# maxwerhahn/Multi-pass-GAN

Measured on AMD Instinct MI355X. Metric: volumes/sec (4x two-pass generator inference, 64^3->256^3 density-only), higher is better.
Workload: dtype f16+2xbf6->f32

## Files before the change

### include/mpgan.h

```cpp
#ifndef MPGAN_H
#define MPGAN_H

#include <stddef.h>
#include <stdint.h>

#ifdef __cplusplus
extern "C" {
#endif

typedef void* mpg_stream_t;

enum { MPG_OK = 0, MPG_ERR_ARG = 1, MPG_ERR_HIP = 2, MPG_ERR_UNSUPPORTED = 3 };

enum { MPG_ACT_NONE = 0, MPG_ACT_RELU = 1, MPG_ACT_LRELU = 2, MPG_ACT_TANH = 3 };

enum { MPG_PREC_F16X1 = 1, MPG_PREC_F16F6 = 2, MPG_PREC_F16X3 = 3 };

enum { MPG_G8_F16 = 0 };

const char* mpg_last_error(void);
int mpg_device_info(int* cu_count, char* arch_name, int arch_name_len);
const char* mpg_version(void);

size_t mpg_g8_bytes(int n, int h, int w, int c);
// ... 31 lines not shown
    float*  y;
    void*   y_g8;
    int32_t prec;
    int32_t reserved;
    const float* in_amax;
} mpg_conv_desc;

size_t mpg_conv_pack_size(int kh, int kw, int cin, int cout, int prec);

int mpg_conv_pack_weights(mpg_stream_t stream, const float* w_hwio, int kh, int kw,
                          int w_cin_total, int w_c_off, int cin, int cout,
                          float wscale, const float* cout_scale,
                          int prec, void* out, size_t out_bytes);

int mpg_conv2d_fused(mpg_stream_t stream, const mpg_conv_desc* desc);

int mpg_conv2d_fused_d2s(mpg_stream_t stream, const mpg_conv_desc* desc, int r, int c_total, int co_off);

int mpg_conv2d_fused_window(mpg_stream_t stream, const mpg_conv_desc* desc, int c_total, int co_off);

typedef struct mpg_small_pair_desc {
    int32_t n, h, w;
    const void* x;
    int32_t cin, cgroups, g_off, up_log2;
    const void* wpack_a;
    int32_t kh_a, kw_a, cmid;
    const float* bias_a;
    int32_t act_a;
    float   leak_a;
    const void* wpack_b;
// ... 179 lines not shown
```

### multi-pass-gan_amd/_lib.py

```python
import ctypes
import os

_HERE = os.path.dirname(os.path.abspath(__file__))
LIB_PATH = os.path.join(_HERE, "csrc", "libmpgan_hip.so")
if os.environ.get("MPGAN_LIB_OVERRIDE"):
    LIB_PATH = os.path.abspath(os.environ["MPGAN_LIB_OVERRIDE"])

MPG_OK = 0
ACT_NONE, ACT_RELU, ACT_LRELU, ACT_TANH = 0, 1, 2, 3
PREC_F16X1, PREC_F16F6, PREC_F16X3 = 1, 2, 3
G8_F16 = 0
MAX_SEG = 4
WGRAD_PLAN_INTS, WGRAD_FORM_ROW, WGRAD_FORM_RING = 24, 0, 1
DEFLATE_UNIT, DEFLATE_SLOT, DEFLATE_SLAB = 32768, 32768 + 16, 64 << 20

_ACT_IDS = {None: ACT_NONE, "none": ACT_NONE, "relu": ACT_RELU, "lrelu": ACT_LRELU, "tanh": ACT_TANH}


def act_id(name):
    try:
        return _ACT_IDS[name]
    except KeyError:
        raise ValueError("unknown activation %r" % (name,))


class MpgError(RuntimeError):
    pass

# ... 63 lines not shown
_Z = ctypes.c_size_t
_F = ctypes.c_float

PROTOTYPES = {
    "mpg_last_error": (ctypes.c_char_p, []),
    "mpg_version": (ctypes.c_char_p, []),
    "mpg_device_info": (_I, [ctypes.POINTER(_I), ctypes.c_char_p, _I]),
    "mpg_g8_bytes": (_Z, [_I, _I, _I, _I]),
    "mpg_f32_to_g8": (_I, [_P, _P, _I, _I, _I, _I, _I, _I, _I, _P]),
    "mpg_f32_to_g8_scaled": (_I, [_P, _P, _I, _I, _I, _I, _I, _I, _I, _P, _P]),
    "mpg_absmax": (_I, [_P, _P, _Z, _P]),
    "mpg_g8_to_f32": (_I, [_P, _P, _I, _I, _I, _I, _P]),
    "mpg_conv_pack_size": (_Z, [_I, _I, _I, _I, _I]),
    "mpg_conv_pack_weights": (_I, [_P, _P, _I, _I, _I, _I, _I, _I, _F, _P, _I, _P, _Z]),
    "mpg_conv2d_fused": (_I, [_P, ctypes.POINTER(ConvDesc)]),
    "mpg_conv2d_fused_d2s": (_I, [_P, ctypes.POINTER(ConvDesc), _I, _I, _I]),
    "mpg_conv2d_fused_window": (_I, [_P, ctypes.POINTER(ConvDesc), _I, _I]),
    "mpg_conv2d_small_pair": (_I, [_P, ctypes.POINTER(SmallPairDesc)]),
    "mpg_conv2d_direct": (_I, [_P, _P, _I, _I, _I, _I, _P, _I, _I, _I, _I, _I, _F, _P, _P, _I, _F, _P]),
    "mpg_resize_nearest": (_I, [_P, _P, _I, _I, _I, _I, _P, _I, _I]),
    "mpg_resize_bilinear": (_I, [_P, _P, _I, _I, _I, _I, _P, _I, _I]),
    "mpg_resize_bicubic": (_I, [_P, _P, _I, _I, _I, _I, _P, _I, _I]),
    "mpg_avg_pool2": (_I, [_P, _P, _I, _I, _I, _I, _P]),
    "mpg_max_pool": (_I, [_P, _P, _I, _I, _I, _I, _I, _I, _P, _P]),
    "mpg_max_pool_bwd": (_I, [_P, _P, _P, _I, _I, _I, _I, _I, _I, _P]),
    "mpg_pixel_norm": (_I, [_P, _P, _Z, _I, _F, _P]),
    "mpg_pixel_norm_g8": (_I, [_P, _P, _I, _I, _I, _I, _F, _P]),
    "mpg_minibatch_stddev": (_I, [_P, _P, _I, _I, _I, _I, _I, _P, _P]),
    "mpg_minibatch_stddev_bwd": (_I, [_P, _P, _P, _I, _I, _I, _I, _I, _P, _P]),
    "mpg_minibatch_stddev_bwd2": (_I, [_P, _P, _P, _P, _I, _I, _I, _I, _I, _P, _P, _P, _Z]),
# ... 94 lines not shown
```

### multi-pass-gan_amd/csrc/mpgan_conv.h

```cpp
#pragma once
#include "mpgan_internal.h"
#include "mpgan_mfma_dev.h"

namespace mpg::conv {

using namespace mpg::dev;

constexpr int TW = 32;
constexpr int TAPOFF_BYTES = 1024;
constexpr int epi_rowf(int nt) { return nt * 32 + 4; }

struct SegArgs {
    const char* x;
    const char* w;
    int cg_seg;
    int cg_total, g_off;
    int kh, kw;
    int up, upy;
    int cgc, nchunks, sc;
    int ih, iw;
    int pt, pl;
    int hs, ws;
    int np;
    int ni_img;
// ... 22 lines not shown
    int tap_bytes;
    int tiles_x, tiles_y;
    int dbg;
};

typedef const __attribute__((address_space(4))) ConvArgs* KArgs;

struct ConvArgsD2S {
    ConvArgs a;
    int cs;
    int coff;
    int cg;
};
typedef const __attribute__((address_space(4))) ConvArgsD2S* KArgsD2S;

template <bool D2S>
struct KernelArgs { typedef ConvArgs type; };
template <>
struct KernelArgs<true> { typedef ConvArgsD2S type; };

struct D2SPos {
    int cc;
    size_t pix;
};
__device__ __forceinline__ D2SPos d2s_pos(const KArgsD2S dp, int py, int px, int c) {
    const int gc = dp->coff + c;
    const int k = gc / dp->cs;
    D2SPos p;
    p.cc = gc - k * dp->cs;
    p.pix = (size_t)(2 * py + (k >> 1)) * (2 * dp->a.w) + 2 * px + (k & 1);
// ... 64 lines not shown
            const int c = (k >> 2) * 8 + 4 * hh + (k & 3);
            stg_lane[c] = c < cout ? tanhf(stg_lane[c]) : 0.f;
        }
#pragma unroll
        for (int nt = 0; nt < NT; ++nt)
#pragma unroll
            for (int q4 = 0; q4 < 4; ++q4) {
                const float4 v = *reinterpret_cast<const float4*>(stg_lane + nt * 32 + 8 * q4 + 4 * hh);
                acc[nt][4 * q4] = v.x;
                acc[nt][4 * q4 + 1] = v.y;
                acc[nt][4 * q4 + 2] = v.z;
                acc[nt][4 * q4 + 3] = v.w;
            }
        return;
    }
    float4 bq[2][4];
#pragma unroll
    for (int q4 = 0; q4 < 4; ++q4) bq[0][q4] = *reinterpret_cast<const float4*>(bl + 8 * q4 + 4 * hh);
#pragma unroll
    for (int nt = 0; nt < NT; ++nt) {
        if (nt + 1 < NT) {
#pragma unroll
            for (int q4 = 0; q4 < 4; ++q4) bq[(nt + 1) & 1][q4] = *reinterpret_cast<const float4*>(bl + (nt + 1) * 32 + 8 * q4 + 4 * hh);
        }
        __builtin_amdgcn_sched_barrier(0);
#pragma unroll
        for (int q4 = 0; q4 < 4; ++q4) {
            const int co0 = nt * 32 + 8 * q4 + 4 * hh;
            const float b4[4] = {bq[nt & 1][q4].x, bq[nt & 1][q4].y, bq[nt & 1][q4].z, bq[nt & 1][q4].w};
#pragma unroll
            for (int i = 0; i < 4; ++i) {
                float v = mpg::apply_act(acc[nt][4 * q4 + i] * unscale + b4[i], ACT, leak);
                if (co0 + i >= cout) v = 0.f;
                acc[nt][4 * q4 + i] = v;
            }
        }
        __builtin_amdgcn_sched_barrier(0);
    }
}

template <int NT>
__device__ __forceinline__ void epilogue_row_values(f32x16 (&acc)[NT], const KArgs ap, const float* bl, float* stg_lane, float unscale,
                                                    int hh) {
    const auto& a = *ap;
    switch (a.act) {
        case MPG_ACT_RELU: epilogue_bias_act<MPG_ACT_RELU>(acc, bl, stg_lane, unscale, a.leak, a.cout, hh); break;
        case MPG_ACT_LRELU: epilogue_bias_act<MPG_ACT_LRELU>(acc, bl, stg_lane, unscale, a.leak, a.cout, hh); break;
        case MPG_ACT_TANH: epilogue_bias_act<MPG_ACT_TANH>(acc, bl, stg_lane, unscale, a.leak, a.cout, hh); break;
        default: epilogue_bias_act<MPG_ACT_NONE>(acc, bl, stg_lane, unscale, a.leak, a.cout, hh); break;
    }
    if (a.pn) {
        float ss = 0.f;
#pragma unroll
        for (int nt = 0; nt < NT; ++nt)
#pragma unroll
            for (int i = 0; i < 16; ++i) ss += acc[nt][i] * acc[nt][i];
        ss += __shfl_xor(ss, 32);
        const float sc = rsqrtf(ss / (float)a.cout + a.pn_eps);
#pragma unroll
        for (int nt = 0; nt < NT; ++nt)
#pragma unroll
            for (int i = 0; i < 16; ++i) acc[nt][i] *= sc;
    }
}

template <int NT, int PT, bool D2S = false>
__device__ __forceinline__ void conv_epilogue(f32x16 (&acc)[PT][NT], const KArgs ap, char* smem, int n, int y0, int x0,
                                              int wave, int lane, const EpiPre pre) {
    const auto& a = *ap;
    const KArgsD2S dp = reinterpret_cast<KArgsD2S>(ap);
    const int r = lane & 31;
    const int hh = lane >> 5;
    constexpr int ROWF = epi_rowf(NT);
    static_assert(128 * sizeof(float) <= TAPOFF_BYTES, "the staged bias must fit in front of the staging rows");
    float* bl = reinterpret_cast<float*>(smem);
    float* stg = reinterpret_cast<float*>(smem + TAPOFF_BYTES) + wave * (32 * ROWF);
    const int cg_out = (a.cout + 7) >> 3;
    const float unscale = 1.f / mpg::pow2_scale(pre.amax);
    {
        float bv = pre.bias;
        asm volatile("" : "+v"(bv));
        if (wave < 2) bl[wave * 64 + lane] = bv;
    }
    __syncthreads();
    const int npx = min(32, a.w - x0);
    const size_t plane_px = (size_t)a.h * a.w;
    if (a.y == nullptr && a.post_add == nullptr) {
#pragma unroll
        for (int pt = 0; pt < PT; ++pt) {
            const int py = y0 + PT * wave + pt;
            epilogue_row_values<NT>(acc[pt], ap, bl, stg + r * ROWF, unscale, hh);
            if (py < a.h && r < npx && !(a.dbg & 2)) {
#pragma unroll
                for (int nt = 0; nt < NT; ++nt)
#pragma unroll
                    for (int qp = 0; qp < 2; ++qp) {
                        float v[8];
#pragma unroll
                        for (int i = 0; i < 4; ++i) {
                            typedef unsigned v2u_t __attribute__((ext_vector_type(2)));
                            const v2u_t sw = __builtin_amdgcn_permlane32_swap(__float_as_uint(acc[pt][nt][8 * qp + i]),
                                                                              __float_as_uint(acc[pt][nt][8 * qp + 4 + i]), false, false);
                            v[i] = __uint_as_float(sw[0]);
                            v[4 + i] = __uint_as_float(sw[1]);
                        }
                        const int cg = nt * 4 + 2 * qp + hh;
                        if (cg < cg_out) {
                            char* dst;
                            size_t plane_out = plane_px;
                            if constexpr (D2S) {
                                const D2SPos q = d2s_pos(dp, py, x0 + r, 8 * cg);
                                plane_out = 4 * plane_px;
                                dst = a.y_g8 + ((((size_t)n * dp->cg + (q.cc >> 3)) * 2) * plane_out + q.pix) * 16;
                            } else {
                                dst = a.y_g8 + ((((size_t)n * a.cg_img + cg) * 2) * plane_px + (size_t)py * a.w + x0 + r) * 16;
                            }
                            half8 hi, lo;
#pragma unroll
                            for (int j = 0; j < 8; ++j) {
                                hi[j] = (_Float16)v[j];
                                lo[j] = (_Float16)(v[j] - (float)hi[j]);
                            }
                            __builtin_nontemporal_store(hi, reinterpret_cast<half8*>(dst));
                            __builtin_nontemporal_store(lo, reinterpret_cast<half8*>(dst + plane_out * 16));
                        }
                    }
            }
        }
        return;
    }
#pragma unroll
    for (int pt = 0; pt < PT; ++pt) {
        const int py = y0 + PT * wave + pt;
        epilogue_row_values<NT>(acc[pt], ap, bl, stg + r * ROWF, unscale, hh);
#pragma unroll
        for (int nt = 0; nt < NT; ++nt)
#pragma unroll
            for (int q4 = 0; q4 < 4; ++q4) {
                const int co0 = nt * 32 + 8 * q4 + 4 * hh;
                *reinterpret_cast<float4*>(stg + r * ROWF + co0) =
                    make_float4(acc[pt][nt][4 * q4], acc[pt][nt][4 * q4 + 1], acc[pt][nt][4 * q4 + 2], acc[pt][nt][4 * q4 + 3]);
            }
        if (py < a.h && !(a.dbg & 2)) {
// ... 99 lines not shown
    int slots;
    int stages;
};
SegShape seg_shape(int kh, int kw, int cin, int nt, int prec);

constexpr size_t LDS_MAX = 160 * 1024;

size_t pack_base_bytes(int kh, int kw, int cin, int cout, int prec);
inline bool small_layer(int cin, int cout) { return cin <= 8 && cout <= 8; }
inline int pad_before(int k, int pad_hi) { return pad_hi ? k / 2 : (k - 1) / 2; }
int check_segment(const mpg_conv_desc* d, int s);

hipError_t launch_conv_f16(int prec, int nt, dim3 grid, size_t lds, hipStream_t st, const ConvArgs& a);
hipError_t launch_conv_f16(int prec, int nt, dim3 grid, size_t lds, hipStream_t st, const ConvArgsD2S& a);
hipError_t launch_conv_f6(int nt, dim3 grid, size_t lds, hipStream_t st, const ConvArgs& a);
int launch_small(hipStream_t stream, const mpg_conv_desc* d);

}
```

### multi-pass-gan_amd/csrc/mpgan_conv_mfma.hip

```cpp
#include "mpgan_conv.h"

using namespace mpg::conv;

namespace {

template <class P>
constexpr Shape shape_of() {
    return {P::TH, P::KS, P::WAVES, P::WSTAGE, P::R * P::WSTAGE, P::ROWF};
}
constexpr Shape SHAPES[3][4] = {
    {shape_of<Pipe<1, 1>>(), shape_of<Pipe<2, 1>>(), shape_of<Pipe<3, 1>>(), shape_of<Pipe<4, 1>>()},
    {shape_of<Pipe6<1>>(), shape_of<Pipe6<2>>(), shape_of<Pipe6<3>>(), shape_of<Pipe6<4>>()},
    {shape_of<Pipe<1, 3>>(), shape_of<Pipe<2, 3>>(), shape_of<Pipe<3, 3>>(), shape_of<Pipe<4, 3>>()},
};
static_assert(MPG_PREC_F16X1 == 1 && MPG_PREC_F16F6 == 2 && MPG_PREC_F16X3 == 3, "SHAPES is indexed by prec - 1");

constexpr size_t LDS_TWO_WG = 80 * 1024;
struct LdsPlan {
    size_t tap, loop, epi, total;
};
LdsPlan lds_plan(int tap_slots, int img_bytes, const Shape& ps) {
    LdsPlan l;
    l.tap = ((size_t)tap_slots * 4 + 1023) / 1024 * 1024;
    if (l.tap < (size_t)TAPOFF_BYTES) l.tap = TAPOFF_BYTES;
// ... 27 lines not shown
    s.stages = s.sc = (s.nchunks * s.tp + stage_slots - 1) / stage_slots;
    s.slots = s.sc * stage_slots;
    s.pref = 1;
    for (int g = 1; g < s.nchunks; ++g)
        if ((g * s.tp) / stage_slots - ((g - 1) * s.tp + stage_slots - 1) / stage_slots < 2) s.pref = 0;
    return s;
}

struct D2SOut {
    int cs, coff;
};

struct WinOut {
    int c_total, co_off;
};

}

const Shape& mpg::conv::pipe_shape(int nt, int prec) { return SHAPES[prec - 1][nt - 1]; }

SegShape mpg::conv::seg_shape(int kh, int kw, int cin, int nt, int prec) {
    if (prec == MPG_PREC_F16F6) return seg_shape_f6(kh, kw, cin, nt);
    const Shape& ps = pipe_shape(nt, prec);
    const int cg = (cin + 7) / 8;
    SegShape s = {};
    set_image(s, ps, kh, kw, 2);
    if (cg < 2 || !((kh * kw) & 1) || lds_plan(0, s.img_bytes, ps).loop > LDS_TWO_WG) set_image(s, ps, kh, kw, 1);
    s.nchunks = (cg + s.cgc - 1) / s.cgc;
    const int ksteps = (kh * kw * s.cgc + 1) / 2;
    s.sc = (ksteps + ps.ks - 1) / ps.ks;
// ... 13 lines not shown

int mpg::conv::check_segment(const mpg_conv_desc* d, int s) {
    const mpg_conv_seg& g = d->seg[s];
    MPG_REQUIRE(g.x && g.wpack, "mpg_conv2d_fused: segment %d null pointer", s);
    MPG_REQUIRE(g.kh >= 1 && g.kh <= 7 && g.kw >= 1 && g.kw <= 7, "mpg_conv2d_fused: segment %d kernel %dx%d", s, g.kh, g.kw);
    MPG_REQUIRE(g.cin >= 1 && g.g_off >= 0 && g.g_off + (g.cin + 7) / 8 <= g.cgroups,
                "mpg_conv2d_fused: segment %d channel-group range", s);
    MPG_REQUIRE(g.up_log2 >= 0 && g.up_log2 <= 4, "mpg_conv2d_fused: segment %d up_log2 %d", s, g.up_log2);
    MPG_REQUIRE(g.up_x_only == 0 || g.up_x_only == 1, "mpg_conv2d_fused: segment %d up_x_only %d (0 or 1)", s, g.up_x_only);
    MPG_REQUIRE((g.up_x_only || (d->h % (1 << g.up_log2)) == 0) && (d->w % (1 << g.up_log2)) == 0,
                "mpg_conv2d_fused: segment %d: %dx%d not divisible by upsample %d", s, d->h, d->w, 1 << g.up_log2);
    MPG_REQUIRE((((uintptr_t)g.x) & 15) == 0 && (((uintptr_t)g.wpack) & 15) == 0, "mpg_conv2d_fused: segment %d misaligned", s);
    return MPG_OK;
}

static int launch_mfma(hipStream_t stream, const mpg_conv_desc* d, const D2SOut* d2s, const WinOut& win) {
    const int nt = (d->cout + 31) / 32;
    const Shape& ps = pipe_shape(nt, d->prec);
    ConvArgs a;
    a.n = d->n; a.h = d->h; a.w = d->w; a.cout = d->cout; a.nseg = d->nseg;
    int max_img = 0, max_slots = 0;
    for (int s = 0; s < d->nseg; ++s) {
        if (const int rc = check_segment(d, s)) return rc;
        const mpg_conv_seg& g = d->seg[s];
        const SegShape ss = seg_shape(g.kh, g.kw, g.cin, nt, d->prec);
        MPG_REQUIRE(d->prec == MPG_PREC_F16F6 || ss.slots <= TAPOFF_BYTES / 4, "mpg_conv2d_fused: segment %d tap table too large", s);
        SegArgs& o = a.seg[s];
        o.x = (const char*)g.x; o.w = (const char*)g.wpack;
        o.cg_seg = (g.cin + 7) / 8; o.cg_total = g.cgroups; o.g_off = g.g_off;
        o.kh = g.kh; o.kw = g.kw; o.up = g.up_log2; o.upy = g.up_x_only ? 0 : g.up_log2;
        o.cgc = ss.cgc; o.nchunks = ss.nchunks; o.sc = ss.sc;
        o.ih = ps.th + g.kh - 1; o.iw = TW + g.kw - 1;
        o.pt = pad_before(g.kh, g.pad_hi); o.pl = pad_before(g.kw, g.pad_hi);
        o.hs = d->h >> o.upy; o.ws = d->w >> o.up;
        o.np = ss.np; o.ni_img = ss.ni_img;
        o.direct = ss.direct;
        o.tp = ss.tp;
        MPG_REQUIRE(!ss.direct || (size_t)o.hs * o.ws * 16 * 16 < ((size_t)1 << 31),
                    "mpg_conv2d_fused: segment %d: %dx%d too large for the 1x1 path (32-bit group offsets)", s, d->h, d->w);
        o.pref = ss.pref;
// ... 6 lines not shown
    MPG_REQUIRE(!d->post_add || d->post_add_coff + d->cout <= d->post_add_stride, "mpg_conv2d_fused: post_add channel range");
    a.y_stride = win.c_total;
    a.cg_img = (win.c_total + 7) / 8;
    a.y = d->y != nullptr ? d->y + win.co_off : nullptr;
    a.y_g8 = d->y_g8 != nullptr ? (char*)d->y_g8 + (size_t)(win.co_off / 8) * 2 * d->h * d->w * 16 : nullptr;
    MPG_REQUIRE((((uintptr_t)d->y) & 15) == 0 && (((uintptr_t)d->y_g8) & 15) == 0,
                "mpg_conv2d_fused: misaligned output");
    a.zeros = mpg::zero_page();
    MPG_REQUIRE(a.zeros != nullptr, "mpg_conv2d_fused: could not allocate the zero page");
    a.img_bytes = max_img;
    a.tiles_x = (d->w + TW - 1) / TW;
    a.tiles_y = (d->h + ps.th - 1) / ps.th;
    a.dbg = d->reserved;
    const long nblk = (long)d->n * a.tiles_x * a.tiles_y;
    MPG_REQUIRE(nblk < (1L << 31), "mpg_conv2d_fused: grid too large");
    const LdsPlan lds = lds_plan(max_slots, max_img, ps);
    a.tap_bytes = (int)lds.tap;
    MPG_REQUIRE(lds.total <= LDS_MAX, "mpg_conv2d_fused: LDS budget %zu exceeds 160 KiB", lds.total);
    const dim3 grid((unsigned)nblk);
    hipError_t le;
    if (d2s != nullptr) {
        ConvArgsD2S ad;
        ad.a = a;
        ad.cs = d2s->cs;
        ad.coff = d2s->coff;
        ad.cg = d2s->cs / 8;
        le = launch_conv_f16(d->prec, nt, grid, lds.total, stream, ad);
    } else if (d->prec == MPG_PREC_F16F6) {
        le = launch_conv_f6(nt, grid, lds.total, stream, a);
    } else {
        le = launch_conv_f16(d->prec, nt, grid, lds.total, stream, a);
    }
    if (le != hipSuccess) return mpg::hip_check(le, "mpg_conv2d_fused: hipFuncSetAttribute(dynamic LDS)");
    MPG_LAUNCH_CHECK("conv_mfma_kernel");
}

static int conv2d_fused(mpg_stream_t stream, const mpg_conv_desc* d, const D2SOut* d2s, const WinOut* window = nullptr) {
    MPG_REQUIRE(d != nullptr, "mpg_conv2d_fused: null desc");
    MPG_REQUIRE(d->n >= 1 && d->h >= 1 && d->w >= 1, "mpg_conv2d_fused: bad shape %d x %d x %d", d->n, d->h, d->w);
    MPG_REQUIRE(d->cout >= 1 && d->cout <= 128, "mpg_conv2d_fused: cout %d not in 1..128", d->cout);
    MPG_REQUIRE(d->nseg >= 1 && d->nseg <= MPG_MAX_SEG, "mpg_conv2d_fused: nseg %d", d->nseg);
    MPG_REQUIRE(d->y != nullptr || d->y_g8 != nullptr, "mpg_conv2d_fused: no output requested");
    MPG_REQUIRE(d->prec == MPG_PREC_F16X1 || d->prec == MPG_PREC_F16X3 || d->prec == MPG_PREC_F16F6,
                "mpg_conv2d_fused: bad prec %d", d->prec);
    MPG_REQUIRE(d->act >= MPG_ACT_NONE && d->act <= MPG_ACT_TANH, "mpg_conv2d_fused: bad act %d", d->act);
    bool small = d->cout <= 8 && !d->pixel_norm && d->post_add == nullptr && d->reserved == 0 && d2s == nullptr && window == nullptr;
    for (int s = 0; s < d->nseg && small; ++s) small = d->seg[s].cin <= 8;
    const WinOut whole = {d->cout, 0};
    return small ? launch_small((hipStream_t)stream, d) : launch_mfma((hipStream_t)stream, d, d2s, window != nullptr ? *window : whole);
}

extern "C" int mpg_conv2d_fused(mpg_stream_t stream, const mpg_conv_desc* d) {
    return conv2d_fused(stream, d, nullptr);
}

extern "C" int mpg_conv2d_fused_d2s(mpg_stream_t stream, const mpg_conv_desc* d, int r, int c_total, int co_off) {
    MPG_REQUIRE(d != nullptr, "mpg_conv2d_fused_d2s: null desc");
    MPG_REQUIRE(r == 2, "mpg_conv2d_fused_d2s: block size %d (only 2)", r);
    MPG_REQUIRE(c_total >= 4 && c_total % 4 == 0, "mpg_conv2d_fused_d2s: %d channels are not a multiple of 4", c_total);
    MPG_REQUIRE(co_off >= 0 && d->cout >= 1 && co_off + d->cout <= c_total,
                "mpg_conv2d_fused_d2s: channels [%d, %d) outside 0..%d", co_off, co_off + d->cout, c_total);
    MPG_REQUIRE(!d->pixel_norm && d->post_add == nullptr, "mpg_conv2d_fused_d2s: no pixel norm or post-add");
    if (d->prec == MPG_PREC_F16F6) {
        mpg::set_error("mpg_conv2d_fused_d2s: MPG_PREC_F16F6 has no depth-to-space store (use MPG_PREC_F16X3 / F16X1)");
// ... 23 lines not shown
```

### multi-pass-gan_amd/csrc/mpgan_mfma_dev.h

```cpp
#pragma once
#include <hip/hip_runtime.h>
#include <type_traits>

namespace mpg::dev {

typedef _Float16 half8 __attribute__((ext_vector_type(8)));
typedef float f32x16 __attribute__((ext_vector_type(16)));

typedef int v4i __attribute__((ext_vector_type(4)));

template <int N>
__device__ __forceinline__ void wait_dma_and_barrier() {
    asm volatile("s_waitcnt vmcnt(%0) lgkmcnt(0)\n\ts_barrier" ::"n"(N) : "memory");
}
__device__ __forceinline__ void wait_dma_late_and_barrier(int late) {
    asm volatile(
        "s_cmp_lt_u32 %0, 1\n\t"
        "s_cbranch_scc1 .Lmpg_w0_%=\n\t"
        "s_cmp_lt_u32 %0, 2\n\t"
        "s_cbranch_scc1 .Lmpg_w1_%=\n\t"
        "s_cmp_lt_u32 %0, 3\n\t"
        "s_cbranch_scc1 .Lmpg_w2_%=\n\t"
        "s_cmp_lt_u32 %0, 4\n\t"
        "s_cbranch_scc1 .Lmpg_w3_%=\n\t"
// ... 50 lines not shown
```

### multi-pass-gan_amd/ops.py

```python
import ctypes

import torch

from . import _lib
from ._lib import G8_F16, PREC_F16F6, PREC_F16X1, PREC_F16X3

DEFAULT_PREC = PREC_F16X3
INFERENCE_PREC = PREC_F16F6
F16F6_MIN_K = 256


def parse_prec(v):
    names = {"f16f6": PREC_F16F6, "f16x3": PREC_F16X3, "f16x1": PREC_F16X1, "fp32": PREC_F16X3}
    s = str(v).strip().lower()
    if s in names:
        return names[s]
    try:
        p = int(s)
    except ValueError:
        p = -1
    if p not in (PREC_F16X1, PREC_F16F6, PREC_F16X3):
        raise _lib.MpgError("prec %r: expected 1 (f16x1), 2 (f16f6) or 3 (f16x3)" % (v,))
    return p

# ... 176 lines not shown
                 in_amax=None):
    lib = _lib.load()
    d = _conv_desc(segments, out_hw, _dev(bias, "bias") if bias is not None else None, act, leak)
    shape = (d.n, d.h, d.w, d.cout)
    d.pixel_norm, d.pn_eps = int(bool(pixel_norm)), pn_eps
    if post_add is not None:
        pa = _checked_post_add(post_add, post_add_coff, shape, "conv2d_fused")
        d.post_add, d.post_add_stride, d.post_add_coff = pa.data_ptr(), pa.shape[3], post_add_coff
    y, y8, outs = _alloc_outputs(shape, segments[0].x.buf.device, want_f32, want_g8, out, "conv2d_fused")
    d.y, d.y_g8 = _ptr(y), _ptr(y8)
    d.reserved = reserved
    if in_amax is not None:
        d.in_amax = _dev(in_amax, "in_amax").data_ptr()
    _lib.check(lib.mpg_conv2d_fused(_stream(), ctypes.byref(d)), "mpg_conv2d_fused")
    return outs[0] if len(outs) == 1 else tuple(outs)


def _launch_windows(what, entry, lead_args, chunks, out_hw, c_total, out_c, bias, act, leak, want_f32, want_g8, out,
                    post_add=None, post_add_coff=0, g8_only=False):
    lib = _lib.load()
    if not chunks:
        raise _lib.MpgError("%s: no chunks" % what)
    co = 0
    for segments, co_off in sorted(chunks, key=lambda ch: ch[1]):
        if co_off != co:
            break
        co += segments[0].packed.cout
    if co != c_total:
        raise _lib.MpgError("%s: the chunks do not cover channels 0..%d once" % (what, c_total))
    if bias is not None:
# ... 504 lines not shown
```

Measured before the change: 15.68.

## Add persistent resident conv kernel with atomic tile scheduler and double-buffered images

Adds a persistent conv kernel launched with one block per compute unit. Each block pulls output tiles from a global atomic counter and double-buffers the input image tile in LDS, so the DMA for the next tile overlaps the MFMA work and epilogue of the current one. The kernel is used automatically for single-segment f16x1/f16x3 convolutions with 96-128 output channels, g8-only output and no tanh or post-add. It also factors the g8 epilogue into a shared helper and exposes plan/kernel-selection entry points for testing. In exchange it adds per-stream counter state that must reset correctly between launches, and a smaller grid that relies on the dynamic scheduler to balance load.

```diff
diff --git a/include/mpgan.h b/include/mpgan.h
--- a/include/mpgan.h
+++ b/include/mpgan.h
@@ -69,6 +69,13 @@
                           int prec, void* out, size_t out_bytes);
 
 int mpg_conv2d_fused(mpg_stream_t stream, const mpg_conv_desc* desc);
+
+#define MPG_CONV_PLAN_INTS 8
+#define MPG_CONV_KERNEL_SMALL 0
+#define MPG_CONV_KERNEL_STREAM 1
+#define MPG_CONV_KERNEL_RESIDENT 2
+int mpg_conv2d_fused_plan(const mpg_conv_desc* desc, int d2s, int32_t* record);
+int mpg_conv2d_fused_kernel(mpg_stream_t stream, const mpg_conv_desc* desc, int kernel, int blocks);
 
 int mpg_conv2d_fused_d2s(mpg_stream_t stream, const mpg_conv_desc* desc, int r, int c_total, int co_off);
 
diff --git a/multi-pass-gan_amd/_lib.py b/multi-pass-gan_amd/_lib.py
--- a/multi-pass-gan_amd/_lib.py
+++ b/multi-pass-gan_amd/_lib.py
@@ -12,6 +12,7 @@
 G8_F16 = 0
 MAX_SEG = 4
 WGRAD_PLAN_INTS, WGRAD_FORM_ROW, WGRAD_FORM_RING = 24, 0, 1
+CONV_PLAN_INTS, CONV_KERNEL_SMALL, CONV_KERNEL_STREAM, CONV_KERNEL_RESIDENT = 8, 0, 1, 2
 DEFLATE_UNIT, DEFLATE_SLOT, DEFLATE_SLAB = 32768, 32768 + 16, 64 << 20
 
 _ACT_IDS = {None: ACT_NONE, "none": ACT_NONE, "relu": ACT_RELU, "lrelu": ACT_LRELU, "tanh": ACT_TANH}
@@ -105,6 +106,8 @@
     "mpg_conv_pack_size": (_Z, [_I, _I, _I, _I, _I]),
     "mpg_conv_pack_weights": (_I, [_P, _P, _I, _I, _I, _I, _I, _I, _F, _P, _I, _P, _Z]),
     "mpg_conv2d_fused": (_I, [_P, ctypes.POINTER(ConvDesc)]),
+    "mpg_conv2d_fused_plan": (_I, [ctypes.POINTER(ConvDesc), _I, ctypes.POINTER(ctypes.c_int32)]),
+    "mpg_conv2d_fused_kernel": (_I, [_P, ctypes.POINTER(ConvDesc), _I, _I]),
     "mpg_conv2d_fused_d2s": (_I, [_P, ctypes.POINTER(ConvDesc), _I, _I, _I]),
     "mpg_conv2d_fused_window": (_I, [_P, ctypes.POINTER(ConvDesc), _I, _I]),
     "mpg_conv2d_small_pair": (_I, [_P, ctypes.POINTER(SmallPairDesc)]),
diff --git a/multi-pass-gan_amd/csrc/mpgan_conv.h b/multi-pass-gan_amd/csrc/mpgan_conv.h
--- a/multi-pass-gan_amd/csrc/mpgan_conv.h
+++ b/multi-pass-gan_amd/csrc/mpgan_conv.h
@@ -60,6 +60,14 @@
 };
 typedef const __attribute__((address_space(4))) ConvArgsD2S* KArgsD2S;
 
+struct ConvArgsRes {
+    ConvArgs a;
+    unsigned* ctr;
+    int ntiles;
+    int nblocks;
+};
+typedef const __attribute__((address_space(4))) ConvArgsRes* KArgsRes;
+
 template <bool D2S>
 struct KernelArgs { typedef ConvArgs type; };
 template <>
@@ -154,14 +162,14 @@
             }
         return;
     }
-    float4 bq[2][4];
-#pragma unroll
-    for (int q4 = 0; q4 < 4; ++q4) bq[0][q4] = *reinterpret_cast<const float4*>(bl + 8 * q4 + 4 * hh);
+    v4f bq[2][4];
+#pragma unroll
+    for (int q4 = 0; q4 < 4; ++q4) bq[0][q4] = *reinterpret_cast<const v4f*>(bl + 8 * q4 + 4 * hh);
 #pragma unroll
     for (int nt = 0; nt < NT; ++nt) {
         if (nt + 1 < NT) {
 #pragma unroll
-            for (int q4 = 0; q4 < 4; ++q4) bq[(nt + 1) & 1][q4] = *reinterpret_cast<const float4*>(bl + (nt + 1) * 32 + 8 * q4 + 4 * hh);
+            for (int q4 = 0; q4 < 4; ++q4) bq[(nt + 1) & 1][q4] = *reinterpret_cast<const v4f*>(bl + (nt + 1) * 32 + 8 * q4 + 4 * hh);
         }
         __builtin_amdgcn_sched_barrier(0);
 #pragma unroll
@@ -179,14 +187,18 @@
     }
 }
 
-template <int NT>
+template <int NT, bool TANH = true>
 __device__ __forceinline__ void epilogue_row_values(f32x16 (&acc)[NT], const KArgs ap, const float* bl, float* stg_lane, float unscale,
                                                     int hh) {
     const auto& a = *ap;
     switch (a.act) {
         case MPG_ACT_RELU: epilogue_bias_act<MPG_ACT_RELU>(acc, bl, stg_lane, unscale, a.leak, a.cout, hh); break;
         case MPG_ACT_LRELU: epilogue_bias_act<MPG_ACT_LRELU>(acc, bl, stg_lane, unscale, a.leak, a.cout, hh); break;
-        case MPG_ACT_TANH: epilogue_bias_act<MPG_ACT_TANH>(acc, bl, stg_lane, unscale, a.leak, a.cout, hh); break;
+        case MPG_ACT_TANH:
+            if constexpr (TANH) {
+                epilogue_bias_act<MPG_ACT_TANH>(acc, bl, stg_lane, unscale, a.leak, a.cout, hh);
+                break;
+            }
         default: epilogue_bias_act<MPG_ACT_NONE>(acc, bl, stg_lane, unscale, a.leak, a.cout, hh); break;
     }
     if (a.pn) {
@@ -201,6 +213,61 @@
         for (int nt = 0; nt < NT; ++nt)
 #pragma unroll
             for (int i = 0; i < 16; ++i) acc[nt][i] *= sc;
+    }
+}
+
+constexpr int epilogue_g8_stores(int nt, int pt) { return pt * nt * 2 * 2; }
+template <int NT, int PT, bool D2S = false, bool TANH = true>
+__device__ __forceinline__ void epilogue_rows_g8(f32x16 (&acc)[PT][NT], const KArgs ap, const float* bl, float* stg, int n, int y0,
+                                                 int x0, int wave, int lane, float unscale) {
+    const auto& a = *ap;
+    const KArgsD2S dp = reinterpret_cast<KArgsD2S>(ap);
+    const int r = lane & 31;
+    const int hh = lane >> 5;
+    constexpr int ROWF = epi_rowf(NT);
+    const int cg_out = (a.cout + 7) >> 3;
+    const int npx = min(32, a.w - x0);
+    const size_t plane_px = (size_t)a.h * a.w;
+#pragma unroll
+    for (int pt = 0; pt < PT; ++pt) {
+        const int py = y0 + PT * wave + pt;
+        epilogue_row_values<NT, TANH>(acc[pt], ap, bl, stg + r * ROWF, unscale, hh);
+        if (py < a.h && r < npx && !(a.dbg & 2)) {
+#pragma unroll
+            for (int nt = 0; nt < NT; ++nt)
+#pragma unroll
+                for (int qp = 0; qp < 2; ++qp) {
+                    float v[8];
+#pragma unroll
+                    for (int i = 0; i < 4; ++i) {
+                        typedef unsigned v2u_t __attribute__((ext_vector_type(2)));
+                        const v2u_t sw = __builtin_amdgcn_permlane32_swap(__float_as_uint(acc[pt][nt][8 * qp + i]),
+                                                                          __float_as_uint(acc[pt][nt][8 * qp + 4 + i]), false, false);
+                        v[i] = __uint_as_float(sw[0]);
+                        v[4 + i] = __uint_as_float(sw[1]);
+                    }
+                    const int cg = nt * 4 + 2 * qp + hh;
+                    if (cg < cg_out) {
+                        char* dst;
+                        size_t plane_out = plane_px;
+                        if constexpr (D2S) {
+                            const D2SPos q = d2s_pos(dp, py, x0 + r, 8 * cg);
+                            plane_out = 4 * plane_px;
+                            dst = a.y_g8 + ((((size_t)n * dp->cg + (q.cc >> 3)) * 2) * plane_out + q.pix) * 16;
+                        } else {
+                            dst = a.y_g8 + ((((size_t)n * a.cg_img + cg) * 2) * plane_px + (size_t)py * a.w + x0 + r) * 16;
+                        }
+                        half8 hi, lo;
+#pragma unroll
+                        for (int j = 0; j < 8; ++j) {
+                            hi[j] = (_Float16)v[j];
+                            lo[j] = (_Float16)(v[j] - (float)hi[j]);
+                        }
+                        __builtin_nontemporal_store(hi, reinterpret_cast<half8*>(dst));
+                        __builtin_nontemporal_store(lo, reinterpret_cast<half8*>(dst + plane_out * 16));
+                    }
+                }
+        }
     }
 }
 
@@ -226,47 +293,7 @@
     const int npx = min(32, a.w - x0);
     const size_t plane_px = (size_t)a.h * a.w;
     if (a.y == nullptr && a.post_add == nullptr) {
-#pragma unroll
-        for (int pt = 0; pt < PT; ++pt) {
-            const int py = y0 + PT * wave + pt;
-            epilogue_row_values<NT>(acc[pt], ap, bl, stg + r * ROWF, unscale, hh);
-            if (py < a.h && r < npx && !(a.dbg & 2)) {
-#pragma unroll
-                for (int nt = 0; nt < NT; ++nt)
-#pragma unroll
-                    for (int qp = 0; qp < 2; ++qp) {
-                        float v[8];
-#pragma unroll
-                        for (int i = 0; i < 4; ++i) {
-                            typedef unsigned v2u_t __attribute__((ext_vector_type(2)));
-                            const v2u_t sw = __builtin_amdgcn_permlane32_swap(__float_as_uint(acc[pt][nt][8 * qp + i]),
-                                                                              __float_as_uint(acc[pt][nt][8 * qp + 4 + i]), false, false);
-                            v[i] = __uint_as_float(sw[0]);
-                            v[4 + i] = __uint_as_float(sw[1]);
-                        }
-                        const int cg = nt * 4 + 2 * qp + hh;
-                        if (cg < cg_out) {
-                            char* dst;
-                            size_t plane_out = plane_px;
-                            if constexpr (D2S) {
-                                const D2SPos q = d2s_pos(dp, py, x0 + r, 8 * cg);
-                                plane_out = 4 * plane_px;
-                                dst = a.y_g8 + ((((size_t)n * dp->cg + (q.cc >> 3)) * 2) * plane_out + q.pix) * 16;
-                            } else {
-                                dst = a.y_g8 + ((((size_t)n * a.cg_img + cg) * 2) * plane_px + (size_t)py * a.w + x0 + r) * 16;
-                            }
-                            half8 hi, lo;
-#pragma unroll
-                            for (int j = 0; j < 8; ++j) {
-                                hi[j] = (_Float16)v[j];
-                                lo[j] = (_Float16)(v[j] - (float)hi[j]);
-                            }
-                            __builtin_nontemporal_store(hi, reinterpret_cast<half8*>(dst));
-                            __builtin_nontemporal_store(lo, reinterpret_cast<half8*>(dst + plane_out * 16));
-                        }
-                    }
-            }
-        }
+        epilogue_rows_g8<NT, PT, D2S>(acc, ap, bl, stg, n, y0, x0, wave, lane, unscale);
         return;
     }
 #pragma unroll
@@ -396,6 +423,10 @@
 hipError_t launch_conv_f16(int prec, int nt, dim3 grid, size_t lds, hipStream_t st, const ConvArgs& a);
 hipError_t launch_conv_f16(int prec, int nt, dim3 grid, size_t lds, hipStream_t st, const ConvArgsD2S& a);
 hipError_t launch_conv_f6(int nt, dim3 grid, size_t lds, hipStream_t st, const ConvArgs& a);
+constexpr int RES_TH = 16, RES_WAVES = 8, RES_CTL_BYTES = 1024;
+unsigned* resident_counters(hipStream_t st);
+int resident_default_blocks();
+hipError_t launch_conv_resident(int prec, int nt, size_t lds, hipStream_t st, const ConvArgsRes& a);
 int launch_small(hipStream_t stream, const mpg_conv_desc* d);
 
 }
diff --git a/multi-pass-gan_amd/csrc/mpgan_conv_mfma.hip b/multi-pass-gan_amd/csrc/mpgan_conv_mfma.hip
--- a/multi-pass-gan_amd/csrc/mpgan_conv_mfma.hip
+++ b/multi-pass-gan_amd/csrc/mpgan_conv_mfma.hip
@@ -65,6 +65,37 @@
 struct WinOut {
     int c_total, co_off;
 };
+
+constexpr int ROUTE_AUTO = -1;
+
+bool small_launch(const mpg_conv_desc* d, bool d2s, bool window) {
+    bool small = d->cout <= 8 && !d->pixel_norm && d->post_add == nullptr && d->reserved == 0 && !d2s && !window;
+    for (int s = 0; s < d->nseg && small; ++s) small = d->seg[s].cin <= 8;
+    return small;
+}
+
+struct ResidentPlan {
+    bool ok;
+    SegShape ss;
+    size_t lds;
+};
+ResidentPlan resident_plan(const mpg_conv_desc* d, bool d2s) {
+    ResidentPlan p = {};
+    const int nt = (d->cout + 31) / 32;
+    if ((d->prec != MPG_PREC_F16X3 && d->prec != MPG_PREC_F16X1) || d->nseg != 1 || d2s || nt < 3 || nt > 4) return p;
+    if (d->y != nullptr || d->y_g8 == nullptr || d->post_add != nullptr || d->act == MPG_ACT_TANH) return p;
+    const mpg_conv_seg& g = d->seg[0];
+    if (g.kh < 1 || g.kh > 7 || g.kw < 1 || g.kw > 7 || g.cin < 1) return p;
+    p.ss = seg_shape(g.kh, g.kw, g.cin, nt, d->prec);
+    if (p.ss.nchunks != 1 || p.ss.slots > TAPOFF_BYTES / 4) return p;
+    Shape tile = pipe_shape(nt, d->prec);
+    tile.th = RES_TH;
+    tile.waves = RES_WAVES;
+    set_image(p.ss, tile, g.kh, g.kw, p.ss.cgc);
+    p.lds = (size_t)TAPOFF_BYTES + RES_CTL_BYTES + (size_t)p.ss.stages * tile.wstage + 2 * (size_t)p.ss.img_bytes;
+    p.ok = p.lds <= LDS_MAX;
+    return p;
+}
 
 }
 
@@ -108,16 +139,26 @@
     return MPG_OK;
 }
 
-static int launch_mfma(hipStream_t stream, const mpg_conv_desc* d, const D2SOut* d2s, const WinOut& win) {
+static int launch_mfma(hipStream_t stream, const mpg_conv_desc* d, const D2SOut* d2s, const WinOut& win, int route = ROUTE_AUTO,
+                       int blocks = 0) {
     const int nt = (d->cout + 31) / 32;
-    const Shape& ps = pipe_shape(nt, d->prec);
+    const ResidentPlan rplan = route == MPG_CONV_KERNEL_STREAM ? ResidentPlan{} : resident_plan(d, d2s != nullptr);
+    MPG_REQUIRE(route != MPG_CONV_KERNEL_RESIDENT || rplan.ok, "mpg_conv2d_fused_kernel: the launch is not eligible for conv_resident_kernel");
+    unsigned* ctr = rplan.ok ? resident_counters(stream) : nullptr;
+    MPG_REQUIRE(route != MPG_CONV_KERNEL_RESIDENT || ctr != nullptr, "mpg_conv2d_fused_kernel: no counter slot for this stream");
+    const bool resident = ctr != nullptr;
+    Shape ps = pipe_shape(nt, d->prec);
+    if (resident) {
+        ps.th = RES_TH;
+        ps.waves = RES_WAVES;
+    }
     ConvArgs a;
     a.n = d->n; a.h = d->h; a.w = d->w; a.cout = d->cout; a.nseg = d->nseg;
     int max_img = 0, max_slots = 0;
     for (int s = 0; s < d->nseg; ++s) {
         if (const int rc = check_segment(d, s)) return rc;
         const mpg_conv_seg& g = d->seg[s];
-        const SegShape ss = seg_shape(g.kh, g.kw, g.cin, nt, d->prec);
+        const SegShape ss = resident ? rplan.ss : seg_shape(g.kh, g.kw, g.cin, nt, d->prec);
         MPG_REQUIRE(d->prec == MPG_PREC_F16F6 || ss.slots <= TAPOFF_BYTES / 4, "mpg_conv2d_fused: segment %d tap table too large", s);
         SegArgs& o = a.seg[s];
         o.x = (const char*)g.x; o.w = (const char*)g.wpack;
@@ -154,6 +195,19 @@
     a.dbg = d->reserved;
     const long nblk = (long)d->n * a.tiles_x * a.tiles_y;
     MPG_REQUIRE(nblk < (1L << 31), "mpg_conv2d_fused: grid too large");
+    if (resident) {
+        ConvArgsRes ar;
+        ar.a = a;
+        ar.a.tap_bytes = TAPOFF_BYTES;
+        ar.ctr = ctr;
+        ar.ntiles = (int)nblk;
+        if (blocks <= 0) blocks = resident_default_blocks();
+        MPG_REQUIRE(blocks > 0, "mpg_conv2d_fused: could not read the device's compute-unit count");
+        ar.nblocks = blocks > nblk ? (int)nblk : blocks;
+        const hipError_t e = launch_conv_resident(d->prec, nt, rplan.lds, stream, ar);
+        if (e != hipSuccess) return mpg::hip_check(e, "mpg_conv2d_fused: hipFuncSetAttribute(dynamic LDS)");
+        MPG_LAUNCH_CHECK("conv_resident_kernel");
+    }
     const LdsPlan lds = lds_plan(max_slots, max_img, ps);
     a.tap_bytes = (int)lds.tap;
     MPG_REQUIRE(lds.total <= LDS_MAX, "mpg_conv2d_fused: LDS budget %zu exceeds 160 KiB", lds.total);
@@ -175,7 +229,7 @@
     MPG_LAUNCH_CHECK("conv_mfma_kernel");
 }
 
-static int conv2d_fused(mpg_stream_t stream, const mpg_conv_desc* d, const D2SOut* d2s, const WinOut* window = nullptr) {
+static int check_desc(const mpg_conv_desc* d) {
     MPG_REQUIRE(d != nullptr, "mpg_conv2d_fused: null desc");
     MPG_REQUIRE(d->n >= 1 && d->h >= 1 && d->w >= 1, "mpg_conv2d_fused: bad shape %d x %d x %d", d->n, d->h, d->w);
     MPG_REQUIRE(d->cout >= 1 && d->cout <= 128, "mpg_conv2d_fused: cout %d not in 1..128", d->cout);
@@ -184,10 +238,56 @@
     MPG_REQUIRE(d->prec == MPG_PREC_F16X1 || d->prec == MPG_PREC_F16X3 || d->prec == MPG_PREC_F16F6,
                 "mpg_conv2d_fused: bad prec %d", d->prec);
     MPG_REQUIRE(d->act >= MPG_ACT_NONE && d->act <= MPG_ACT_TANH, "mpg_conv2d_fused: bad act %d", d->act);
-    bool small = d->cout <= 8 && !d->pixel_norm && d->post_add == nullptr && d->reserved == 0 && d2s == nullptr && window == nullptr;
-    for (int s = 0; s < d->nseg && small; ++s) small = d->seg[s].cin <= 8;
+    return MPG_OK;
+}
+
+static int conv2d_fused(mpg_stream_t stream, const mpg_conv_desc* d, const D2SOut* d2s, const WinOut* window = nullptr) {
+    if (const int rc = check_desc(d)) return rc;
     const WinOut whole = {d->cout, 0};
-    return small ? launch_small((hipStream_t)stream, d) : launch_mfma((hipStream_t)stream, d, d2s, window != nullptr ? *window : whole);
+    return small_launch(d, d2s != nullptr, window != nullptr) ? launch_small((hipStream_t)stream, d)
+                                                              : launch_mfma((hipStream_t)stream, d, d2s, window != nullptr ? *window : whole);
+}
+
+extern "C" int mpg_conv2d_fused_plan(const mpg_conv_desc* d, int d2s, int32_t* record) {
+    if (const int rc = check_desc(d)) return rc;
+    MPG_REQUIRE(record != nullptr, "mpg_conv2d_fused_plan: null record");
+    for (int i = 0; i < MPG_CONV_PLAN_INTS; ++i) record[i] = 0;
+    if (small_launch(d, d2s != 0, false)) {
+        record[0] = MPG_CONV_KERNEL_SMALL;
+        return MPG_OK;
+    }
+    const int nt = (d->cout + 31) / 32;
+    const ResidentPlan rp = resident_plan(d, d2s != 0);
+    const Shape& ps = pipe_shape(nt, d->prec);
+    const int th = rp.ok ? RES_TH : ps.th;
+    record[0] = rp.ok ? MPG_CONV_KERNEL_RESIDENT : MPG_CONV_KERNEL_STREAM;
+    record[1] = nt;
+    record[2] = th;
+    record[3] = rp.ok ? RES_WAVES : ps.waves;
+    const long tiles = (long)d->n * ((d->h + th - 1) / th) * ((d->w + TW - 1) / TW);
+    MPG_REQUIRE(tiles < (1L << 31), "mpg_conv2d_fused: grid too large");
+    record[4] = (int32_t)tiles;
+    if (rp.ok) {
+        record[5] = (int32_t)rp.lds;
+    } else {
+        int max_img = 0, max_slots = 0;
+        for (int s = 0; s < d->nseg; ++s) {
+            if (const int rc = check_segment(d, s)) return rc;
+            const SegShape ss = seg_shape(d->seg[s].kh, d->seg[s].kw, d->seg[s].cin, nt, d->prec);
+            max_img = ss.img_bytes > max_img ? ss.img_bytes : max_img;
+            max_slots = ss.slots > max_slots ? ss.slots : max_slots;
+        }
+        record[5] = (int32_t)lds_plan(max_slots, max_img, ps).total;
+    }
+    return MPG_OK;
+}
+
+extern "C" int mpg_conv2d_fused_kernel(mpg_stream_t stream, const mpg_conv_desc* d, int kernel, int blocks) {
+    if (const int rc = check_desc(d)) return rc;
+    MPG_REQUIRE(kernel == MPG_CONV_KERNEL_STREAM || kernel == MPG_CONV_KERNEL_RESIDENT, "mpg_conv2d_fused_kernel: kernel %d", kernel);
+    MPG_REQUIRE(blocks >= 0, "mpg_conv2d_fused_kernel: blocks %d", blocks);
+    const WinOut whole = {d->cout, 0};
+    return launch_mfma((hipStream_t)stream, d, nullptr, whole, kernel, blocks);
 }
 
 extern "C" int mpg_conv2d_fused(mpg_stream_t stream, const mpg_conv_desc* d) {
diff --git a/multi-pass-gan_amd/csrc/mpgan_conv_resident.hip b/multi-pass-gan_amd/csrc/mpgan_conv_resident.hip
--- /dev/null
+++ b/multi-pass-gan_amd/csrc/mpgan_conv_resident.hip
@@ -0,0 +1,264 @@
+#include <mutex>
+
+#include "mpgan_conv.h"
+
+using namespace mpg::conv;
+
+namespace {
+
+template <int N>
+__device__ __forceinline__ void wait_counted_and_barrier(int counted) {
+    static_assert(N >= 0 && N < 64, "vmcnt has six bits");
+    asm volatile(
+        "s_cmp_eq_u32 %0, 0\n\t"
+        "s_cbranch_scc1 .Lmpg_rz_%=\n\t"
+        "s_waitcnt vmcnt(%1)\n\t"
+        "s_branch .Lmpg_rb_%=\n"
+        ".Lmpg_rz_%=:\n\t"
+        "s_waitcnt vmcnt(0)\n"
+        ".Lmpg_rb_%=:\n\t"
+        "s_waitcnt lgkmcnt(0)\n\t"
+        "s_barrier" ::"s"(__builtin_amdgcn_readfirstlane(counted)), "n"(N)
+        : "memory", "scc");
+}
+
+template <int NT, int PREC>
+__global__ __launch_bounds__(RES_WAVES * 64, 2) void conv_resident_kernel(const ConvArgsRes a_unused) {
+    extern __shared__ __attribute__((aligned(16))) char smem[];
+    const KArgs ap = (KArgs)__builtin_amdgcn_kernarg_segment_ptr();
+    const KArgsRes rp = reinterpret_cast<KArgsRes>(ap);
+    const auto& a = *ap;
+    const auto& sg = ap->seg[0];
+    using P = Pipe<NT, PREC>;
+    constexpr int PT = RES_TH / RES_WAVES, TH = RES_TH, KS = P::KS, WPLANE = P::WPLANE, WSTAGE = P::WSTAGE;
+    constexpr int THREADS = RES_WAVES * 64;
+    static_assert(PT == 2, "two tile rows per wave");
+    static_assert(128 * sizeof(float) + 2 * sizeof(int) <= RES_CTL_BYTES, "staged bias and two tickets");
+
+    int* tapoff = reinterpret_cast<int*>(smem);
+    float* bl = reinterpret_cast<float*>(smem + TAPOFF_BYTES);
+    int* tk = reinterpret_cast<int*>(smem + TAPOFF_BYTES + 512);
+    char* w_lds = smem + TAPOFF_BYTES + RES_CTL_BYTES;
+    const int nk = sg.sc * KS;
+    const int wbytes = sg.sc * WSTAGE;
+    char* img_lds = w_lds + wbytes;
+
+    const int tid = threadIdx.x;
+    const int lane = tid & 63;
+    const int wave = tid >> 6;
+    const int wave_u = __builtin_amdgcn_readfirstlane(wave);
+    const int r = lane & 31;
+    const int hh = lane >> 5;
+    const int ntiles = rp->ntiles;
+
+    auto draw = [&]() {
+        unsigned z = 0;
+        asm volatile("" : "+v"(z));
+        return atomicAdd(rp->ctr + z, 1u);
+    };
+    unsigned drawn = 0;
+    if (tid == 0) drawn = draw();
+
+    const int CGC = sg.cgc;
+    const int TG = sg.kh * sg.kw * CGC;
+    const int plane_b = sg.np * 16;
+    const int group_b = plane_b * 2;
+    const int ppg = sg.np >> 6;
+    int pixb[PT];
+#pragma unroll
+    for (int pt = 0; pt < PT; ++pt) pixb[pt] = ((PT * wave + pt) * sg.iw + r) * 16;
+
+    auto tile_at = [&](int t, int& n, int& y0, int& x0) {
+        const int tx = t % a.tiles_x;
+        const int t2 = t / a.tiles_x;
+        const int ty = t2 % a.tiles_y;
+        n = t2 / a.tiles_y;
+        y0 = ty * TH;
+        x0 = tx * TW;
+    };
+    const size_t plane_px = (size_t)sg.hs * sg.ws;
+    auto dma_image = [&](int tile, int b) {
+        int n, y0, x0;
+        tile_at(tile, n, y0, x0);
+        char* buf = img_lds + b * a.img_bytes;
+        for (int i = 0; i < sg.ni_img; ++i) {
+            const int pc = RES_WAVES * i + wave_u;
+            const int g = pc / (2 * ppg);
+            const int rem = pc - g * 2 * ppg;
+            const int pl = rem / ppg;
+            const int p = (rem - pl * ppg) * 64 + lane;
+            const int hy = p / sg.iw;
+            const int hx = p - hy * sg.iw;
+            const int yy = y0 - sg.pt + hy;
+            const int xx = x0 - sg.pl + hx;
+            const char* src = a.zeros;
+            if (g < CGC && g < sg.cg_seg && hy < sg.ih && yy >= 0 && yy < a.h && xx >= 0 && xx < a.w && (PREC == 3 || pl == 0))
+                src = sg.x + ((((size_t)n * sg.cg_total + sg.g_off + g) * 2 + pl) * plane_px + (size_t)(yy >> sg.upy) * sg.ws +
+                              (xx >> sg.up)) * 16;
+            dma16(src, buf + pc * 1024);
+        }
+    };
+
+    int cur = blockIdx.x;
+    int b = 0;
+    dma_image(cur, 0);
+    for (int o = wave_u * 1024; o < wbytes; o += RES_WAVES * 1024) dma16(sg.w + o + lane * 16, w_lds + o);
+    for (int q = tid; q < nk * 2; q += THREADS) {
+        int off = 0;
+        if (q < TG) {
+            const int tap = q / CGC;
+            const int g = q - tap * CGC;
+            const int dy = tap / sg.kw;
+            const int dx = tap - dy * sg.kw;
+            off = (dy * sg.iw + dx) * 16 + g * group_b;
+        }
+        tapoff[q] = off;
+    }
+    {
+        const EpiPre pre = epilogue_prefetch(ap, tid);
+        if (tid < 128) bl[tid] = pre.bias;
+    }
+    const float unscale = 1.f / mpg::pow2_scale(a.in_amax != nullptr ? *a.in_amax : 0.f);
+    if (tid == 0) tk[1] = rp->nblocks + (int)drawn;
+    int counted = 0;
+    for (;;) {
+        wait_counted_and_barrier<epilogue_g8_stores(NT, PT)>(counted);
+        int n, y0, x0;
+        tile_at(cur, n, y0, x0);
+        const int nxt = __builtin_amdgcn_readfirstlane(tk[b ^ 1]);
+        if (nxt < ntiles) {
+            if (tid == 0) drawn = draw();
+            dma_image(nxt, b ^ 1);
+        }
+
+        f32x16 acc[PT][NT];
+#pragma unroll
+        for (int pt = 0; pt < PT; ++pt)
+#pragma unroll
+            for (int nt = 0; nt < NT; ++nt)
+#pragma unroll
+                for (int i = 0; i < 16; ++i) acc[pt][nt][i] = 0.f;
+
+        if (!(a.dbg & 1)) {
+            const char* img = img_lds + b * a.img_bytes;
+            struct Head {
+                half8 b_hi[PT], b_lo[PT], a_hi, a_lo;
+            };
+            auto weights = [&](int kk) {
+                const int st = kk / KS;
+                return w_lds + st * WSTAGE + ((kk - st * KS) * NT * 64 + lane) * 16;
+            };
+            auto load_head = [&](Head& f, int kk) {
+                const int toff = tapoff[2 * kk + hh];
+                const char* wb = weights(kk);
+#pragma unroll
+                for (int pt = 0; pt < PT; ++pt) {
+                    f.b_hi[pt] = *reinterpret_cast<const half8*>(img + pixb[pt] + toff);
+                    if (PREC == 3) f.b_lo[pt] = *reinterpret_cast<const half8*>(img + plane_b + pixb[pt] + toff);
+                }
+                f.a_hi = *reinterpret_cast<const half8*>(wb);
+                if (PREC == 3) f.a_lo = *reinterpret_cast<const half8*>(wb + WPLANE);
+            };
+            auto kstep = [&](const Head& f, int kk) {
+                const char* wb = weights(kk);
+                half8 a_hi[NT], a_lo[NT];
+                a_hi[0] = f.a_hi;
+                a_lo[0] = f.a_lo;
+#pragma unroll
+                for (int nt = 1; nt < NT; ++nt) {
+                    a_hi[nt] = *reinterpret_cast<const half8*>(wb + nt * 1024);
+                    if (PREC == 3) a_lo[nt] = *reinterpret_cast<const half8*>(wb + WPLANE + nt * 1024);
+                }
+#pragma unroll
+                for (int nt = 0; nt < NT; ++nt)
+#pragma unroll
+                    for (int pt = 0; pt < PT; ++pt) {
+                        acc[pt][nt] = __builtin_amdgcn_mfma_f32_32x32x16_f16(a_hi[nt], f.b_hi[pt], acc[pt][nt], 0, 0, 0);
+                        if (PREC == 3) {
+                            acc[pt][nt] = __builtin_amdgcn_mfma_f32_32x32x16_f16(a_lo[nt], f.b_hi[pt], acc[pt][nt], 0, 0, 0);
+                            acc[pt][nt] = __builtin_amdgcn_mfma_f32_32x32x16_f16(a_hi[nt], f.b_lo[pt], acc[pt][nt], 0, 0, 0);
+                        }
+                    }
+            };
+            Head h0, h1;
+            load_head(h0, 0);
+#pragma nounroll
+            for (int kk = 0; kk < nk; kk += 2) {
+                load_head(h1, min(kk + 1, nk - 1));
+                kstep(h0, kk);
+                if (kk + 1 < nk) {
+                    load_head(h0, min(kk + 2, nk - 1));
+                    kstep(h1, kk + 1);
+                }
+            }
+        }
+        if (nxt < ntiles && tid == 0) tk[b] = rp->nblocks + (int)drawn;
+
+        epilogue_rows_g8<NT, PT, false, false>(acc, ap, bl, nullptr, n, y0, x0, wave, lane, unscale);
+        counted = (y0 + TH <= a.h && x0 + TW <= a.w && ((a.cout + 7) >> 3) == NT * 4 && !(a.dbg & 2)) ? 1 : 0;
+        if (nxt >= ntiles) break;
+        cur = nxt;
+        b ^= 1;
+    }
+    if (tid == 0) {
+        const unsigned done = atomicAdd(rp->ctr + 1, 1u);
+        if (done == (unsigned)rp->nblocks - 1) {
+            atomicExch(rp->ctr, 0u);
+            atomicExch(rp->ctr + 1, 0u);
+        }
+    }
+}
+
+constexpr int SLOTS = 256;
+constexpr int SLOT_WORDS = 32;
+struct DeviceSlots {
+    unsigned* base = nullptr;
+    int used = 0;
+    hipStream_t stream[SLOTS];
+};
+
+}
+
+unsigned* mpg::conv::resident_counters(hipStream_t st) {
+    static std::mutex mu;
+    static DeviceSlots per_dev[64];
+    int dev = 0;
+    if (hipGetDevice(&dev) != hipSuccess || dev < 0 || dev >= 64) return nullptr;
+    std::lock_guard<std::mutex> lock(mu);
+    DeviceSlots& ds = per_dev[dev];
+    if (ds.base == nullptr) {
+        unsigned* p = nullptr;
+        const size_t bytes = (size_t)SLOTS * SLOT_WORDS * sizeof(unsigned);
+        if (hipMalloc(&p, bytes) != hipSuccess) return nullptr;
+        if (hipMemset(p, 0, bytes) != hipSuccess || hipDeviceSynchronize() != hipSuccess) {
+            (void)hipFree(p);
+            return nullptr;
+        }
+        ds.base = p;
+    }
+    for (int i = 0; i < ds.used; ++i)
+        if (ds.stream[i] == st) return ds.base + (size_t)i * SLOT_WORDS;
+    if (ds.used == SLOTS) return nullptr;
+    ds.stream[ds.used] = st;
+    return ds.base + (size_t)(ds.used++) * SLOT_WORDS;
+}
+
+int mpg::conv::resident_default_blocks() {
+    static int per_dev[64] = {0};
+    int dev = 0;
+    if (hipGetDevice(&dev) != hipSuccess || dev < 0 || dev >= 64) return 0;
+    int cu = __atomic_load_n(&per_dev[dev], __ATOMIC_RELAXED);
+    if (cu > 0) return cu;
+    if (hipDeviceGetAttribute(&cu, hipDeviceAttributeMultiprocessorCount, dev) != hipSuccess || cu < 1) return 0;
+    __atomic_store_n(&per_dev[dev], cu, __ATOMIC_RELAXED);
+    return cu;
+}
+
+hipError_t mpg::conv::launch_conv_resident(int prec, int nt, size_t lds, hipStream_t st, const ConvArgsRes& a) {
+    const dim3 grid((unsigned)a.nblocks), block(RES_WAVES * 64);
+    if (prec == MPG_PREC_F16X3)
+        return nt == 3 ? mpg::launch_dyn_lds<conv_resident_kernel<3, 3>>(grid, block, lds, st, a)
+                       : mpg::launch_dyn_lds<conv_resident_kernel<4, 3>>(grid, block, lds, st, a);
+    return nt == 3 ? mpg::launch_dyn_lds<conv_resident_kernel<3, 1>>(grid, block, lds, st, a)
+                   : mpg::launch_dyn_lds<conv_resident_kernel<4, 1>>(grid, block, lds, st, a);
+}
diff --git a/multi-pass-gan_amd/csrc/mpgan_mfma_dev.h b/multi-pass-gan_amd/csrc/mpgan_mfma_dev.h
--- a/multi-pass-gan_amd/csrc/mpgan_mfma_dev.h
+++ b/multi-pass-gan_amd/csrc/mpgan_mfma_dev.h
@@ -8,6 +8,7 @@
 typedef float f32x16 __attribute__((ext_vector_type(16)));
 
 typedef int v4i __attribute__((ext_vector_type(4)));
+typedef float v4f __attribute__((ext_vector_type(4)));
 
 template <int N>
 __device__ __forceinline__ void wait_dma_and_barrier() {
diff --git a/multi-pass-gan_amd/ops.py b/multi-pass-gan_amd/ops.py
--- a/multi-pass-gan_amd/ops.py
+++ b/multi-pass-gan_amd/ops.py
@@ -214,6 +214,30 @@
         d.in_amax = _dev(in_amax, "in_amax").data_ptr()
     _lib.check(lib.mpg_conv2d_fused(_stream(), ctypes.byref(d)), "mpg_conv2d_fused")
     return outs[0] if len(outs) == 1 else tuple(outs)
+
+
+def conv2d_fused_plan(segments, out_hw, bias=None, act=None, want_f32=False, want_g8=True, d2s=False):
+    lib = _lib.load()
+    d = _conv_desc(segments, out_hw, bias, act, 0.2)
+    d.y, d.y_g8 = ctypes.c_void_p(16 if want_f32 else 0), ctypes.c_void_p(16 if want_g8 else 0)
+    rec = (ctypes.c_int32 * _lib.CONV_PLAN_INTS)()
+    _lib.check(lib.mpg_conv2d_fused_plan(ctypes.byref(d), int(bool(d2s)), rec), "mpg_conv2d_fused_plan")
+    return dict(zip(("kernel", "nt", "tile_h", "waves", "tiles", "lds_bytes"), rec[:6]))
+
+
+def conv2d_fused_kernel(segments, out_hw, kernel, blocks=0, bias=None, act=None, leak=0.2, pixel_norm=False, pn_eps=1e-8,
+                        in_amax=None, reserved=0):
+    lib = _lib.load()
+    d = _conv_desc(segments, out_hw, _dev(bias, "bias") if bias is not None else None, act, leak)
+    d.pixel_norm, d.pn_eps = int(bool(pixel_norm)), pn_eps
+    y8 = G8.empty(d.n, d.h, d.w, d.cout, segments[0].x.buf.device, G8_F16)
+    y8.buf.fill_(float("nan"))
+    d.y_g8 = _ptr(y8)
+    d.reserved = reserved
+    if in_amax is not None:
+        d.in_amax = _dev(in_amax, "in_amax").data_ptr()
+    _lib.check(lib.mpg_conv2d_fused_kernel(_stream(), ctypes.byref(d), int(kernel), int(blocks)), "mpg_conv2d_fused_kernel")
+    return y8
 
 
 def _launch_windows(what, entry, lead_args, chunks, out_hw, c_total, out_c, bias, act, leak, want_f32, want_g8, out,
```

New measurement: 15.82 (median of 6 runs). About the same (+0.9%).
